# oxylusengine/Oxylus

Measured on NVIDIA H100. Metric: meshlet_instances_culled_per_s, higher is better.
Workload: dtype f32

## Files before the change

oxylus_b200/csrc/kernels_tri.cuh:

```cuda
#pragma once
#include <climits>

#include "oxc_exact.cuh"
#include "oxc_raster_core.cuh"
#include "oxc_tma.cuh"

namespace oxc {

#ifndef OXC_TRI_THREADS
#define OXC_TRI_THREADS 256
#endif
constexpr int TRI_THREADS = OXC_TRI_THREADS;
constexpr int TRI_WARPS = TRI_THREADS / 32;

struct TriParams {
  const OxcMeshletInstance* meshlet_instances;
  const InstCull* inst;
  const InstGeom* geom;
  const OxcMeshletInstanceVisibility* vis;
  const OxcDispatchIndirectCommand* tri_cmd;
  const uint32_t* visible_indices;
  const uint32_t* id_base;
  uint32_t late;
  uint32_t* reordered_indices;
// ... 72 lines not shown
  const uint32_t first = p.late ? p.vis->early_visible_meshlet_instances : 0u;
  const uint32_t count = p.tri_cmd->x;
  const uint32_t id_base = p.id_base ? __ldg(p.id_base) : 0u;
  const uint32_t n_tiles = (count + TRI_WARPS - 1) / TRI_WARPS;
  float4* clip_s = clip_all[warp];
  for (uint32_t tile = blockIdx.x; tile < n_tiles; tile += gridDim.x) {
    const uint32_t g = tile * TRI_WARPS + warp;
    bool pass[2] = {false, false};
    uint32_t rank[2] = {0, 0}, wtotal = 0, data_id = 0;
    if (g < count) {
      const MeshletWork w = load_meshlet(p, first + g, id_base, clip_s, lane);
      data_id = w.data_id;
#pragma unroll
      for (int k = 0; k < 2; k++) {
        const uint32_t t = lane + 32u * k;
        float4 c0, c1, c2;
        pass[k] = t < w.tri_count && triangle_passes(w, t, clip_s, c0, c1, c2);
        if (pass[k] && p.small_primitive_cull && tri_covers_no_sample(c0, c1, c2, p.f_width, p.f_height, p.width, p.height)) pass[k] = false;
        const uint32_t bal = __ballot_sync(0xffffffffu, pass[k]);
        rank[k] = wtotal + __popc(bal & ((1u << lane) - 1u));
        wtotal += __popc(bal);
      }
      __syncwarp();
    }
    if (lane == 0) warp_cnt[warp] = wtotal;
    __syncthreads();
    if (threadIdx.x == 0) {
      uint32_t s = 0;
#pragma unroll
      for (int k = 0; k < TRI_WARPS; k++) { const uint32_t c = warp_cnt[k]; warp_cnt[k] = s; s += c; }
      base_s = s ? atomicAdd(&p.draw_cmd->index_count, s * 3u) : 0u;
    }
    __syncthreads();
    const uint32_t wbase = base_s + warp_cnt[warp] * 3u;
#pragma unroll
    for (int k = 0; k < 2; k++)
      if (pass[k]) {
        const uint32_t t = lane + 32u * k, off = wbase + rank[k] * 3u, masked = data_id << OXC_VIS_PRIMITIVE_BITS;
        p.reordered_indices[off + 0] = masked | ((t * 3u + 0u) & OXC_VIS_PRIMITIVE_MASK);
        p.reordered_indices[off + 1] = masked | ((t * 3u + 1u) & OXC_VIS_PRIMITIVE_MASK);
        p.reordered_indices[off + 2] = masked | ((t * 3u + 2u) & OXC_VIS_PRIMITIVE_MASK);
      }
    __syncthreads();
  }
}

#ifndef OXC_RASTER_MIN_BLOCKS
#define OXC_RASTER_MIN_BLOCKS 3
#endif
#ifndef OXC_RASTER_BIG_PIXELS
#define OXC_RASTER_BIG_PIXELS 32
#endif
#ifndef OXC_RASTER_BATCH
#define OXC_RASTER_BATCH 8
#endif
constexpr int MICRO_STAGE_BYTES = 224;
constexpr int RASTER_BATCH = OXC_RASTER_BATCH;
static_assert(RASTER_BATCH >= 1 && RASTER_BATCH <= 32, "one header per lane: a grab holds at most 32 meshlets");
constexpr int RASTER_BIG_PIXELS = OXC_RASTER_BIG_PIXELS;

struct MeshletHeader {
  uint32_t gid, inst, vertex_offset, vertex_count, tri_offset, tri_count;
  const uint32_t* micro;
  const uint32_t* vidx;
  const uint2* pos;
};

OXC_DI MeshletHeader fetch_header(const TriParams& p, uint32_t slot, uint32_t id_base) {
  MeshletHeader h;
  h.gid = __ldg(&p.visible_indices[slot]);
  const uint2 mi = __ldg(reinterpret_cast<const uint2*>(p.meshlet_instances) + (h.gid - id_base));
  const InstGeom* g = p.geom + mi.x;
  const uint4 g0 = __ldg(reinterpret_cast<const uint4*>(g));
  const uint4 g1 = __ldg(reinterpret_cast<const uint4*>(g) + 1);
  const OxcMeshlet* meshlets = reinterpret_cast<const OxcMeshlet*>(((uint64_t)g0.y << 32) | g0.x);
  const uint4 m = __ldg(reinterpret_cast<const uint4*>(meshlets + mi.y));
  h.inst = mi.x;
  h.vertex_offset = m.x;
  h.tri_offset = m.y;
  h.vertex_count = min(m.z, (uint32_t)OXC_MESHLET_MAX_VERTICES);
  h.tri_count = min(m.w, (uint32_t)OXC_MESHLET_MAX_PRIMITIVES);
  h.micro = reinterpret_cast<const uint32_t*>(((uint64_t)g0.w << 32) | g0.z);
  h.vidx = reinterpret_cast<const uint32_t*>(((uint64_t)g1.y << 32) | g1.x) + m.x;
  h.pos = reinterpret_cast<const uint2*>(((uint64_t)g1.w << 32) | g1.z);
  return h;
}

OXC_DI MeshletHeader bcast_header(const MeshletHeader& h, int src) {
  MeshletHeader o;
  o.gid = __shfl_sync(0xffffffffu, h.gid, src); o.inst = __shfl_sync(0xffffffffu, h.inst, src);
  o.vertex_offset = 0;
  o.vertex_count = __shfl_sync(0xffffffffu, h.vertex_count, src);
  o.tri_offset = __shfl_sync(0xffffffffu, h.tri_offset, src); o.tri_count = __shfl_sync(0xffffffffu, h.tri_count, src);
  o.micro = reinterpret_cast<const uint32_t*>(__shfl_sync(0xffffffffu, reinterpret_cast<unsigned long long>(h.micro), src));
  o.vidx = reinterpret_cast<const uint32_t*>(__shfl_sync(0xffffffffu, reinterpret_cast<unsigned long long>(h.vidx), src));
  o.pos = reinterpret_cast<const uint2*>(__shfl_sync(0xffffffffu, reinterpret_cast<unsigned long long>(h.pos), src));
  return o;
}

constexpr int BIG_CHUNK_W = 64, BIG_CHUNK_H = 32;

OXC_DI void big_entry_store(uint4* dst, const TriSetup& s, int px0, int px1, int py0, int py1, uint32_t data) {
  dst[0] = make_uint4((uint32_t)s.ax, (uint32_t)s.ay, (uint32_t)s.bx, (uint32_t)s.by);
  dst[1] = make_uint4((uint32_t)s.cx, (uint32_t)s.cy, __float_as_uint(s.za), __float_as_uint(s.dzb));
  dst[2] = make_uint4(__float_as_uint(s.dzc), (uint32_t)px0, (uint32_t)px1, (uint32_t)py0);
  dst[3] = make_uint4((uint32_t)py1, (uint32_t)s.bias, data, 0u);
}

OXC_DI void big_entry_load(const uint4* src, TriSetup& s, uint32_t& data) {
  const uint4 a = src[0], b = src[1], c = src[2], d = src[3];
  s.ax = (int)a.x; s.ay = (int)a.y; s.bx = (int)a.z; s.by = (int)a.w;
  s.cx = (int)b.x; s.cy = (int)b.y; s.za = __uint_as_float(b.z); s.dzb = __uint_as_float(b.w);
  s.dzc = __uint_as_float(c.x); s.px0 = (int)c.y; s.px1 = (int)c.z; s.py0 = (int)c.w;
  s.py1 = (int)d.x; s.bias = (int)d.y; s.narrow = false;
  data = d.z;
}

OXC_DI bool big_push(const TriParams& p, const TriSetup& s, uint32_t data) {
  if (*reinterpret_cast<volatile uint32_t*>(&p.big_counters[0]) >= p.big_capacity) return false;
  const uint32_t cw = (uint32_t)(s.px1 - s.px0) / BIG_CHUNK_W + 1u, ch = (uint32_t)(s.py1 - s.py0) / BIG_CHUNK_H + 1u;
  const uint32_t n = cw * ch;
  const uint32_t base = atomicAdd(&p.big_counters[0], n);
  if (base >= p.big_capacity) return false;
  if (base + n > p.big_capacity) {
    for (uint32_t k = base; k < p.big_capacity; k++) big_entry_store(p.big_queue + (size_t)k * 4, s, 1, 0, 1, 0, data);
    return false;
  }
  uint32_t k = base;
  for (uint32_t cy = 0; cy < ch; cy++)
    for (uint32_t cx = 0; cx < cw; cx++, k++) {
      const int x0 = s.px0 + (int)(cx * BIG_CHUNK_W), y0 = s.py0 + (int)(cy * BIG_CHUNK_H);
      big_entry_store(p.big_queue + (size_t)k * 4, s, x0, min(s.px1, x0 + BIG_CHUNK_W - 1), y0, min(s.py1, y0 + BIG_CHUNK_H - 1), data);
    }
  return true;
}

constexpr uint32_t BIG_PUSH_ALONE = 4;
OXC_DI uint32_t big_chunk_count(const TriSetup& s) {
  return ((uint32_t)(s.px1 - s.px0) / BIG_CHUNK_W + 1u) * ((uint32_t)(s.py1 - s.py0) / BIG_CHUNK_H + 1u);
}

OXC_DI bool big_push_warp(const TriParams& p, const TriSetup& s, uint32_t data, uint32_t lane) {
  const uint32_t cw = (uint32_t)(s.px1 - s.px0) / BIG_CHUNK_W + 1u, ch = (uint32_t)(s.py1 - s.py0) / BIG_CHUNK_H + 1u;
  const uint32_t n = cw * ch;
  uint32_t base = 0xFFFFFFFFu;
  if (lane == 0 && *reinterpret_cast<volatile uint32_t*>(&p.big_counters[0]) < p.big_capacity) base = atomicAdd(&p.big_counters[0], n);
  base = __shfl_sync(0xffffffffu, base, 0);
  if (base >= p.big_capacity) return false;
  if (base + n > p.big_capacity) {
    for (uint32_t k = base + lane; k < p.big_capacity; k += 32) big_entry_store(p.big_queue + (size_t)k * 4, s, 1, 0, 1, 0, data);
    return false;
  }
  for (uint32_t k = lane; k < n; k += 32) {
    const uint32_t cy = k / cw, cx = k - cy * cw;
    const int x0 = s.px0 + (int)(cx * BIG_CHUNK_W), y0 = s.py0 + (int)(cy * BIG_CHUNK_H);
    big_entry_store(p.big_queue + (size_t)(base + k) * 4, s, x0, min(s.px1, x0 + BIG_CHUNK_W - 1), y0, min(s.py1, y0 + BIG_CHUNK_H - 1), data);
  }
  return true;
}

__global__ void __launch_bounds__(256) k_raster_big(const __grid_constant__ TriParams p) {
  const uint32_t lane = threadIdx.x & 31;
  const uint32_t total = min(p.big_counters[0], p.big_capacity);
  const int lx = lane & 7, ly = lane >> 3;
  for (uint32_t i = blockIdx.x * (blockDim.x >> 5) + (threadIdx.x >> 5); i < total; i += gridDim.x * (blockDim.x >> 5)) {
    TriSetup b;
    uint32_t data;
    big_entry_load(p.big_queue + (size_t)i * 4, b, data);
    for (int ty = b.py0; ty <= b.py1; ty += 4)
      for (int tx = b.px0; tx <= b.px1; tx += 8) {
        const int px = tx + lx, py = ty + ly;
        if (px <= b.px1 && py <= b.py1) raster_pixel(b, px, py, data, p.visbuf, p.width);
      }
  }
}

template <bool PREFETCH_GRAB>
__global__ void __launch_bounds__(TRI_THREADS, OXC_RASTER_MIN_BLOCKS) k_raster_visbuffer(const __grid_constant__ TriParams p) {
  __shared__ float4 clip_all[TRI_WARPS][OXC_MESHLET_MAX_VERTICES];
  __shared__ ScreenVert scr_all[TRI_WARPS][OXC_MESHLET_MAX_VERTICES];
  const uint32_t lane = threadIdx.x & 31, warp = threadIdx.x >> 5;
#ifndef OXC_RASTER_NO_SMEM_MICRO
#define OXC_RASTER_SMEM_MICRO 1
#endif
#ifdef OXC_RASTER_SMEM_MICRO
  __shared__ uint32_t micro_w[TRI_WARPS][52];
#endif
#ifdef OXC_RASTER_TMA_MICRO
  __shared__ __align__(16) uint8_t micro_all[TRI_WARPS][MICRO_STAGE_BYTES];
  __shared__ __align__(8) uint64_t micro_bar[TRI_WARPS];
  if (lane == 0) { mbar_init(&micro_bar[warp], 1); mbar_fence_init(); }
  __syncwarp();
  uint32_t micro_phase = 0;
#endif
  const uint32_t first = p.late ? p.vis->early_visible_meshlet_instances : 0u;
  const uint32_t count = p.tri_cmd->x;
  const uint32_t id_base = p.id_base ? __ldg(p.id_base) : 0u;
  float4* clip_s = clip_all[warp];
  ScreenVert* scr_s = scr_all[warp];
  uint32_t kept = 0;
#ifdef OXC_RASTER_STATS
  unsigned long long t_entry, t_chase = 0, t_proc = 0, n_done = 0, n_grabs = 0;
  asm volatile("mov.u64 %0, %%globaltimer;" : "=l"(t_entry));
#endif
  const uint32_t n_warps2 = gridDim.x * TRI_WARPS * 2u;
  uint32_t g_next = 0, batch_next = 1;
  if (PREFETCH_GRAB && lane == 0) {
    batch_next = min((uint32_t)RASTER_BATCH, max(1u, count / n_warps2));
    g_next = atomicAdd(p.work_counter, batch_next);
  }
  for (;;) {
    uint32_t g0 = 0, batch = 1;
    if (PREFETCH_GRAB) {
      g0 = __shfl_sync(0xffffffffu, g_next, 0);
      batch = __shfl_sync(0xffffffffu, batch_next, 0);
      if (g0 >= count) break;
      if (lane == 0) {
        const uint32_t seen = g0 + batch;
        const uint32_t rem = count > seen ? count - seen : 0u;
        batch_next = min((uint32_t)RASTER_BATCH, max(1u, rem / n_warps2));
        g_next = atomicAdd(p.work_counter, batch_next);
      }
    } else {
      if (lane == 0) {
        const uint32_t seen = *reinterpret_cast<volatile uint32_t*>(p.work_counter);
        const uint32_t rem = count > seen ? count - seen : 0u;
        batch = min((uint32_t)RASTER_BATCH, max(1u, rem / n_warps2));
        g0 = atomicAdd(p.work_counter, batch);
      }
      g0 = __shfl_sync(0xffffffffu, g0, 0);
      batch = __shfl_sync(0xffffffffu, batch, 0);
      if (g0 >= count) break;
    }
    const uint32_t nb = min(batch, count - g0);
    const uint32_t my_survivor = g0 + lane;
#ifdef OXC_RASTER_STATS
    unsigned long long t_a, t_b, t_c;
    asm volatile("mov.u64 %0, %%globaltimer;" : "=l"(t_a));
#endif
    MeshletHeader mine;
    mine.gid = 0; mine.inst = 0; mine.vertex_offset = 0; mine.vertex_count = 0; mine.tri_offset = 0; mine.tri_count = 0;
    mine.micro = nullptr; mine.vidx = nullptr; mine.pos = nullptr;
    if (lane < nb) mine = fetch_header(p, first + my_survivor, id_base);
    MeshletHeader cur = bcast_header(mine, 0);
    uint32_t vi0 = lane < cur.vertex_count ? __ldg(&cur.vidx[lane]) : 0u;
    uint32_t vi1 = lane + 32u < cur.vertex_count ? __ldg(&cur.vidx[lane + 32u]) : 0u;
#ifdef OXC_RASTER_STATS
    if (vi0 + vi1 == 0xFFFFFFFFu) kept++;
    asm volatile("mov.u64 %0, %%globaltimer;" : "=l"(t_b));
#endif
    for (uint32_t j = 0; j < nb; j++) {
      const MeshletHeader w = cur;
#ifdef OXC_RASTER_TMA_MICRO
      const uint64_t micro_addr = reinterpret_cast<uint64_t>(w.micro) + w.tri_offset;
      const uint32_t micro_skew = (uint32_t)(micro_addr & 15u);
      if (lane == 0) {
        const uint32_t bytes = (micro_skew + w.tri_count * 3u + 15u) & ~15u;
        mbar_expect_tx(&micro_bar[warp], bytes);
        tma_load_1d(micro_all[warp], reinterpret_cast<const void*>(micro_addr - micro_skew), bytes, &micro_bar[warp]);
      }
#endif
#ifdef OXC_RASTER_SMEM_MICRO
      {
        const uint32_t n_words = ((w.tri_offset & 3u) + w.tri_count * 3u + 3u) >> 2;
        const uint32_t* src = w.micro + (w.tri_offset >> 2);
        const uint32_t m0 = lane < n_words ? __ldg(src + lane) : 0u;
        const uint32_t m1 = lane + 32u < n_words ? __ldg(src + lane + 32u) : 0u;
        micro_w[warp][lane] = m0;
        if (lane < 20) micro_w[warp][lane + 32] = m1;
      }
#endif
      const uint2 q0 = lane < w.vertex_count ? __ldg(&w.pos[vi0]) : make_uint2(0, 0);
      const uint2 q1 = lane + 32u < w.vertex_count ? __ldg(&w.pos[vi1]) : make_uint2(0, 0);
      if (j + 1 < nb) {
        cur = bcast_header(mine, (int)(j + 1));
        vi0 = lane < cur.vertex_count ? __ldg(&cur.vidx[lane]) : 0u;
        vi1 = lane + 32u < cur.vertex_count ? __ldg(&cur.vidx[lane + 32u]) : 0u;
      }
      const InstCull* ic = p.inst + w.inst;
      const float4 r0 = __ldg(&ic->mvp_row[0]), r1 = __ldg(&ic->mvp_row[1]), r2 = __ldg(&ic->mvp_row[2]), r3 = __ldg(&ic->mvp_row[3]);
      {
        const float x = dequantize_half_hw(q0.x & 0xFFFFu), y = dequantize_half_hw(q0.x >> 16), z = dequantize_half_hw(q0.y & 0xFFFFu);
        const float4 c = make_float4(row_dot_p1(r0, x, y, z), row_dot_p1(r1, x, y, z), row_dot_p1(r2, x, y, z), row_dot_p1(r3, x, y, z));
        clip_s[lane] = c;
        scr_s[lane] = to_screen(c, p.f_width, p.f_height);
      }
      if (w.vertex_count > 32u) {
        const float x = dequantize_half_hw(q1.x & 0xFFFFu), y = dequantize_half_hw(q1.x >> 16), z = dequantize_half_hw(q1.y & 0xFFFFu);
        const float4 c = make_float4(row_dot_p1(r0, x, y, z), row_dot_p1(r1, x, y, z), row_dot_p1(r2, x, y, z), row_dot_p1(r3, x, y, z));
        clip_s[lane + 32] = c;
        scr_s[lane + 32] = to_screen(c, p.f_width, p.f_height);
      }
      __syncwarp();
#ifdef OXC_RASTER_TMA_MICRO
      mbar_wait(&micro_bar[warp], micro_phase);
      micro_phase ^= 1u;
      const uint8_t* micro_s = micro_all[warp] + micro_skew;
#endif
      const uint32_t rounds = (w.tri_count + 31u) >> 5;
      for (uint32_t k = 0; k < rounds; k++) {
        const uint32_t t = lane + 32u * k;
        bool pass = false;
        TriSetup s;
        bool draw = false;
        if (t < w.tri_count) {
#ifdef OXC_RASTER_TMA_MICRO
          const uint32_t i0 = micro_s[t * 3u + 0u], i1 = micro_s[t * 3u + 1u], i2 = micro_s[t * 3u + 2u];
#elif defined(OXC_RASTER_SMEM_MICRO)
          const uint8_t* mb = reinterpret_cast<const uint8_t*>(micro_w[warp]) + (w.tri_offset & 3u) + t * 3u;
          const uint32_t i0 = mb[0], i1 = mb[1], i2 = mb[2];
#else
          const uint32_t base = w.tri_offset + t * 3u;
          const uint32_t i0 = micro_index(w.micro, base + 0u), i1 = micro_index(w.micro, base + 1u), i2 = micro_index(w.micro, base + 2u);
#endif
          if (max(i0, max(i1, i2)) < w.vertex_count) {
            const float4 c0 = clip_s[i0], c1 = clip_s[i1], c2 = clip_s[i2];
            pass = c0.z >= 0.0f && c1.z >= 0.0f && c2.z >= 0.0f && !triangle_backface(c0, c1, c2);
            if (pass) {
              const int why = tri_setup(scr_s[i0], scr_s[i1], scr_s[i2], p.width, p.height, s);
              draw = why == TRI_DRAW;
              if (why == TRI_NO_SAMPLE && p.small_primitive_cull) pass = false;
              if (why == TRI_INVALID_VERTEX && p.clip_queue) {
                const uint32_t slot = atomicAdd(p.clip_counter, 1u);
                if (slot < p.clip_capacity) p.clip_queue[slot] = (w.gid << p.prim_bits) | t;
                else atomicOr(p.status, (uint32_t)OXC_STATUS_CLIP_OVERFLOW);
              }
            }
          }
        }
        kept += pass ? 1u : 0u;
        const uint32_t data = (w.gid << p.prim_bits) | t;
        const int bw = draw ? s.px1 - s.px0 + 1 : 0, bh = draw ? s.py1 - s.py0 + 1 : 0;
#if defined(OXC_RASTER_STATS) && OXC_RASTER_STATS == 1
        {
          const int area = (draw && bw * bh <= RASTER_BIG_PIXELS) ? bw * bh : 0;
          const int mx = __reduce_max_sync(0xffffffffu, area), sm = __reduce_add_sync(0xffffffffu, area);
          const int nd = __popc(__ballot_sync(0xffffffffu, area > 0));
          const int nbig = __popc(__ballot_sync(0xffffffffu, draw && bw * bh > RASTER_BIG_PIXELS));
          if (lane == 0) {
            unsigned long long* st = reinterpret_cast<unsigned long long*>(p.big_queue) + (size_t)p.big_capacity * 8 + (p.late ? 64 : 0);
            atomicAdd(&st[min(mx, 33)], 1ull);
            atomicAdd(&st[40], (unsigned long long)sm);
            atomicAdd(&st[41], (unsigned long long)mx);
            atomicAdd(&st[42], (unsigned long long)nd);
            atomicAdd(&st[43], 1ull);
            atomicAdd(&st[44], (unsigned long long)nbig);
          }
        }
#endif
        bool big = draw && (bw * bh > RASTER_BIG_PIXELS);
        if (draw && !big) raster_small(s, data, p.visbuf, p.width);
        const bool few = big && big_chunk_count(s) <= BIG_PUSH_ALONE;
        if (few && p.big_queue && big_push(p, s, data)) big = false;
        uint32_t big_mask = __ballot_sync(0xffffffffu, big);
        while (big_mask) {
          const int src = __ffs(big_mask) - 1;
          big_mask &= big_mask - 1;
          TriSetup b;
          b.ax = __shfl_sync(0xffffffffu, s.ax, src); b.ay = __shfl_sync(0xffffffffu, s.ay, src);
          b.bx = __shfl_sync(0xffffffffu, s.bx, src); b.by = __shfl_sync(0xffffffffu, s.by, src);
          b.cx = __shfl_sync(0xffffffffu, s.cx, src); b.cy = __shfl_sync(0xffffffffu, s.cy, src);
          b.za = __shfl_sync(0xffffffffu, s.za, src); b.dzb = __shfl_sync(0xffffffffu, s.dzb, src);
          b.dzc = __shfl_sync(0xffffffffu, s.dzc, src);
          b.px0 = __shfl_sync(0xffffffffu, s.px0, src); b.px1 = __shfl_sync(0xffffffffu, s.px1, src);
          b.py0 = __shfl_sync(0xffffffffu, s.py0, src); b.py1 = __shfl_sync(0xffffffffu, s.py1, src);
          b.bias = __shfl_sync(0xffffffffu, s.bias, src);
          const uint32_t bdata = __shfl_sync(0xffffffffu, data, src);
          if (p.big_queue && big_push_warp(p, b, bdata, lane)) continue;
          const int lx = lane & 7, ly = lane >> 3;
          for (int ty = b.py0; ty <= b.py1; ty += 4)
            for (int tx = b.px0; tx <= b.px1; tx += 8) {
              const int px = tx + lx, py = ty + ly;
              if (px <= b.px1 && py <= b.py1) raster_pixel(b, px, py, bdata, p.visbuf, p.width);
            }
        }
      }
      __syncwarp();
    }
#ifdef OXC_RASTER_STATS
    asm volatile("mov.u64 %0, %%globaltimer;" : "=l"(t_c));
    t_chase += t_b - t_a; t_proc += t_c - t_b; n_done += nb; n_grabs++;
#endif
  }
#ifdef OXC_RASTER_STATS
  if (lane == 0) {
    unsigned long long t_exit;
    asm volatile("mov.u64 %0, %%globaltimer;" : "=l"(t_exit));
    unsigned long long* rec = reinterpret_cast<unsigned long long*>(p.big_queue) + (size_t)p.big_capacity * 8 + 128 +
                              ((size_t)(p.late ? gridDim.x * TRI_WARPS : 0) + blockIdx.x * TRI_WARPS + warp) * 6;
    rec[0] = t_entry; rec[1] = t_exit; rec[2] = t_chase; rec[3] = t_proc; rec[4] = n_done; rec[5] = n_grabs;
    if (blockIdx.x == 0 && warp == 0)
      reinterpret_cast<unsigned long long*>(p.big_queue)[(size_t)p.big_capacity * 8 + (p.late ? 64 : 0) + 45] = gridDim.x;
  }
#endif
#pragma unroll
  for (int o = 16; o > 0; o >>= 1) kept += __shfl_xor_sync(0xffffffffu, kept, o);
  if (lane == 0 && kept) atomicAdd(p.tri_counter, (unsigned long long)kept);
}

OXC_DI void clip_and_draw(const TriParams& p, float4 c0, float4 c1, float4 c2, uint32_t data, float fW, float fH) {
  float4 poly[2][12];
  int cur;
  const int n = clip_polygon(c0, c1, c2, poly, cur);
  for (int i = 1; i + 1 < n; i++) {
    TriSetup s;
    if (tri_setup(to_screen(poly[cur][0], fW, fH), to_screen(poly[cur][i], fW, fH), to_screen(poly[cur][i + 1], fW, fH), p.width, p.height, s) != TRI_DRAW)
      continue;
    const int bw = s.px1 - s.px0 + 1, bh = s.py1 - s.py0 + 1;
    if (bw * bh > RASTER_BIG_PIXELS && p.big_queue && big_push(p, s, data)) continue;
    s.narrow = false;
    raster_small(s, data, p.visbuf, p.width);
  }
}

__global__ void __launch_bounds__(128) k_raster_clip_queue(const __grid_constant__ TriParams p) {
  const uint32_t n = min(*p.clip_counter, p.clip_capacity);
  const uint32_t id_base = p.id_base ? __ldg(p.id_base) : 0u;
  for (uint32_t e = blockIdx.x * blockDim.x + threadIdx.x; e < n; e += gridDim.x * blockDim.x) {
    const uint32_t data = p.clip_queue[e];
    const uint32_t gid = data >> p.prim_bits, t = data & ((1u << p.prim_bits) - 1u);
    const uint2 mi = __ldg(reinterpret_cast<const uint2*>(p.meshlet_instances) + (gid - id_base));
    const InstGeom* g = p.geom + mi.x;
    const InstCull* ic = p.inst + mi.x;
    const uint4 m = __ldg(reinterpret_cast<const uint4*>(g->meshlets + mi.y));
    const float4 r0 = __ldg(&ic->mvp_row[0]), r1 = __ldg(&ic->mvp_row[1]), r2 = __ldg(&ic->mvp_row[2]), r3 = __ldg(&ic->mvp_row[3]);
    float4 c[3];
#pragma unroll
    for (int k = 0; k < 3; k++) {
      const uint32_t li = micro_index(g->local_triangle_indices, m.y + t * 3u + k);
      const uint32_t vi = __ldg(&g->indirect_vertex_indices[m.x + li]);
      const uint2 q = __ldg(&g->vertex_positions[vi]);
      const float x = dequantize_half_hw(q.x & 0xFFFFu), y = dequantize_half_hw(q.x >> 16), z = dequantize_half_hw(q.y & 0xFFFFu);
      c[k] = make_float4(row_dot_p1(r0, x, y, z), row_dot_p1(r1, x, y, z), row_dot_p1(r2, x, y, z), row_dot_p1(r3, x, y, z));
    }
    clip_and_draw(p, c[0], c[1], c[2], data, p.f_width, p.f_height);
// ... 55 lines not shown
```

oxylus_b200/csrc/oxc_raster_core.cuh:

```cuda
#pragma once
#include <climits>

#include "oxc_exact.cuh"

namespace oxc {

struct __align__(16) ScreenVert {
  int fx, fy;
  float z;
  int pad;
};

OXC_DI ScreenVert to_screen(float4 c, float fW, float fH) {
  ScreenVert v;
  v.fx = INT_MIN; v.fy = 0; v.z = 0.f; v.pad = 0;
  if (!(c.w > 0.0f)) return v;
  const float rw = fd(1.0f, c.w);
  const float nx = fm(c.x, rw), ny = fm(c.y, rw);
  const float sx = fm(fa(fm(nx, 0.5f), 0.5f), fW), sy = fm(fa(fm(ny, 0.5f), 0.5f), fH);
  const float qx = floorf(fa(fm(sx, 256.0f), 0.5f)), qy = floorf(fa(fm(sy, 256.0f), 0.5f));
  if (!(fabsf(qx) <= 4194304.0f && fabsf(qy) <= 4194304.0f)) return v;
  v.fx = (int)qx; v.fy = (int)qy; v.z = fm(c.z, rw);
  return v;
}

OXC_DI bool tri_covers_no_sample(float4 c0, float4 c1, float4 c2, float fW, float fH, uint32_t W, uint32_t H) {
  const ScreenVert v0 = to_screen(c0, fW, fH), v1 = to_screen(c1, fW, fH), v2 = to_screen(c2, fW, fH);
  if (v0.fx == INT_MIN || v1.fx == INT_MIN || v2.fx == INT_MIN) return false;
  const int minx = min(v0.fx, min(v1.fx, v2.fx)), maxx = max(v0.fx, max(v1.fx, v2.fx));
  const int miny = min(v0.fy, min(v1.fy, v2.fy)), maxy = max(v0.fy, max(v1.fy, v2.fy));
  const int px0 = max(0, (minx - 128 + 255) >> 8), px1 = min((int)W - 1, (maxx - 128) >> 8);
  const int py0 = max(0, (miny - 128 + 255) >> 8), py1 = min((int)H - 1, (maxy - 128) >> 8);
  return px1 < px0 || py1 < py0;
}

struct TriSetup {
  int ax, ay, bx, by, cx, cy;
  float za, dzb, dzc;
  int px0, px1, py0, py1;
  int bias;
  bool narrow;
};

OXC_DI long long orient2d(int ax, int ay, int bx, int by, int cx, int cy) {
  return (long long)(bx - ax) * (long long)(cy - ay) - (long long)(by - ay) * (long long)(cx - ax);
}
OXC_DI int edge_bias_bit(int ax, int ay, int bx, int by) {
  const int dx = bx - ax, dy = by - ay;
  return ((dy > 0) || (dy == 0 && dx < 0)) ? 0 : 1;
}

enum : int { TRI_DRAW = 0, TRI_INVALID_VERTEX = 1, TRI_NO_SAMPLE = 2, TRI_BACK_OR_DEGENERATE = 3 };
OXC_DI int tri_setup(const ScreenVert v0, const ScreenVert v1, const ScreenVert v2, uint32_t W, uint32_t H, TriSetup& s) {
  if (v0.fx == INT_MIN || v1.fx == INT_MIN || v2.fx == INT_MIN) return TRI_INVALID_VERTEX;
  const int minx = min(v0.fx, min(v1.fx, v2.fx)), maxx = max(v0.fx, max(v1.fx, v2.fx));
  const int miny = min(v0.fy, min(v1.fy, v2.fy)), maxy = max(v0.fy, max(v1.fy, v2.fy));
  s.px0 = max(0, (minx - 128 + 255) >> 8);
  s.px1 = min((int)W - 1, (maxx - 128) >> 8);
  s.py0 = max(0, (miny - 128 + 255) >> 8);
  s.py1 = min((int)H - 1, (maxy - 128) >> 8);
  if (s.px1 < s.px0 || s.py1 < s.py0) return TRI_NO_SAMPLE;
  s.narrow = (maxx - minx) < 16384 && (maxy - miny) < 16384;
  long long area2;
  if (s.narrow) area2 = (long long)((v1.fx - v0.fx) * (v2.fy - v0.fy) - (v1.fy - v0.fy) * (v2.fx - v0.fx));
  else area2 = orient2d(v0.fx, v0.fy, v1.fx, v1.fy, v2.fx, v2.fy);
  if (area2 >= 0) return TRI_BACK_OR_DEGENERATE;
  s.ax = v0.fx; s.ay = v0.fy; s.bx = v2.fx; s.by = v2.fy; s.cx = v1.fx; s.cy = v1.fy;
  const float fa_ = (float)(-area2);
  s.za = v0.z;
  s.dzb = fd(fs(v2.z, v0.z), fa_);
  s.dzc = fd(fs(v1.z, v0.z), fa_);
  s.bias = edge_bias_bit(s.bx, s.by, s.cx, s.cy) | (edge_bias_bit(s.cx, s.cy, s.ax, s.ay) << 1) |
           (edge_bias_bit(s.ax, s.ay, s.bx, s.by) << 2);
  return TRI_DRAW;
}

OXC_DI void shade_pixel(const TriSetup& s, long long e0, long long e1, long long e2, int px, int py, uint32_t data,
                        unsigned long long* vis, uint32_t W) {
  if ((e0 - (s.bias & 1)) < 0 || (e1 - ((s.bias >> 1) & 1)) < 0 || (e2 - ((s.bias >> 2) & 1)) < 0) return;
  const float zz = fa(fa(s.za, fm((float)e1, s.dzb)), fm((float)e2, s.dzc));
  if (!(zz >= 0.0f && zz <= 1.0f)) return;
  uint32_t zb = __float_as_uint(zz);
  zb = zb == 0x80000000u ? 0u : zb;
  const unsigned long long v = ((unsigned long long)zb << 32) | data;
  unsigned long long* ptr = vis + (size_t)py * W + px;
  atomicMax(ptr, v);
}

OXC_DI void raster_pixel(const TriSetup& s, int px, int py, uint32_t data, unsigned long long* vis, uint32_t W) {
  const int sx = px * 256 + 128, sy = py * 256 + 128;
  shade_pixel(s, orient2d(s.bx, s.by, s.cx, s.cy, sx, sy), orient2d(s.cx, s.cy, s.ax, s.ay, sx, sy),
              orient2d(s.ax, s.ay, s.bx, s.by, sx, sy), px, py, data, vis, W);
}

OXC_DI int orient2d_32(int ax, int ay, int bx, int by, int cx, int cy) { return (bx - ax) * (cy - ay) - (by - ay) * (cx - ax); }

OXC_DI void shade_pixel_32(const TriSetup& s, int e0, int e1, int e2, int px, int py, uint32_t data, unsigned long long* vis,
                           uint32_t W) {
  if ((e0 - (s.bias & 1)) < 0 || (e1 - ((s.bias >> 1) & 1)) < 0 || (e2 - ((s.bias >> 2) & 1)) < 0) return;
  const float zz = fa(fa(s.za, fm((float)e1, s.dzb)), fm((float)e2, s.dzc));
  if (!(zz >= 0.0f && zz <= 1.0f)) return;
  uint32_t zb = __float_as_uint(zz);
  zb = zb == 0x80000000u ? 0u : zb;
  const unsigned long long v = ((unsigned long long)zb << 32) | data;
  unsigned long long* ptr = vis + (size_t)py * W + px;
  atomicMax(ptr, v);
}

OXC_DI void raster_small(const TriSetup& s, uint32_t data, unsigned long long* vis, uint32_t W) {
  const int sx0 = s.px0 * 256 + 128, sy0 = s.py0 * 256 + 128;
  if (s.narrow) {
    int r0 = orient2d_32(s.bx, s.by, s.cx, s.cy, sx0, sy0), r1 = orient2d_32(s.cx, s.cy, s.ax, s.ay, sx0, sy0),
        r2 = orient2d_32(s.ax, s.ay, s.bx, s.by, sx0, sy0);
    const int dx0 = -(s.cy - s.by) * 256, dy0 = (s.cx - s.bx) * 256, dx1 = -(s.ay - s.cy) * 256, dy1 = (s.ax - s.cx) * 256,
              dx2 = -(s.by - s.ay) * 256, dy2 = (s.bx - s.ax) * 256;
    for (int py = s.py0; py <= s.py1; py++) {
      int e0 = r0, e1 = r1, e2 = r2;
      for (int px = s.px0; px <= s.px1; px++) {
        shade_pixel_32(s, e0, e1, e2, px, py, data, vis, W);
        e0 += dx0; e1 += dx1; e2 += dx2;
      }
      r0 += dy0; r1 += dy1; r2 += dy2;
    }
    return;
  }
  long long r0 = orient2d(s.bx, s.by, s.cx, s.cy, sx0, sy0);
  long long r1 = orient2d(s.cx, s.cy, s.ax, s.ay, sx0, sy0);
  long long r2 = orient2d(s.ax, s.ay, s.bx, s.by, sx0, sy0);
  const long long dx0 = -(long long)(s.cy - s.by) * 256, dy0 = (long long)(s.cx - s.bx) * 256;
  const long long dx1 = -(long long)(s.ay - s.cy) * 256, dy1 = (long long)(s.ax - s.cx) * 256;
  const long long dx2 = -(long long)(s.by - s.ay) * 256, dy2 = (long long)(s.bx - s.ax) * 256;
  for (int py = s.py0; py <= s.py1; py++) {
    long long e0 = r0, e1 = r1, e2 = r2;
    for (int px = s.px0; px <= s.px1; px++) {
      shade_pixel(s, e0, e1, e2, px, py, data, vis, W);
      e0 += dx0; e1 += dx1; e2 += dx2;
    }
    r0 += dy0; r1 += dy1; r2 += dy2;
  }
}

OXC_DI float clip_plane_distance(const float4 v, int plane) {
  switch (plane) {
    case 0: return fs(v.w, v.z);
    case 1: return fa(v.w, v.x);
    case 2: return fs(v.w, v.x);
    case 3: return fa(v.w, v.y);
    default: return fs(v.w, v.y);
  }
}

OXC_DI int clip_polygon(float4 c0, float4 c1, float4 c2, float4 (*poly)[12], int& cur) {
  int n = 3;
  cur = 0;
  poly[0][0] = c0; poly[0][1] = c1; poly[0][2] = c2;
  for (int plane = 0; plane < 5 && n >= 3; plane++) {
    const float4* in = poly[cur];
    float4* out = poly[cur ^ 1];
    int m = 0;
    for (int i = 0; i < n; i++) {
      const float4 A = in[i], B = in[(i + 1) % n];
      const float dA = clip_plane_distance(A, plane), dB = clip_plane_distance(B, plane);
      const bool inA = dA >= 0.0f, inB = dB >= 0.0f;
      if (inA) out[m++] = A;
      if (inA != inB) {
        const float4 I = inA ? A : B, O = inA ? B : A;
        const float dI = inA ? dA : dB, dO = inA ? dB : dA;
        const float tt = fd(dI, fs(dI, dO));
        out[m++] = make_float4(fa(I.x, fm(tt, fs(O.x, I.x))), fa(I.y, fm(tt, fs(O.y, I.y))), fa(I.z, fm(tt, fs(O.z, I.z))),
                               fa(I.w, fm(tt, fs(O.w, I.w))));
      }
    }
    n = m;
    cur ^= 1;
  }
  return n;
}

// ... 2 lines not shown
```

Baseline: 1.808 billion.

## Compact drawable triangles into per-warp shared queue before rasterizing

Drawable triangles are no longer rasterized in the same lane that classified them. Their screen vertices go into a per-warp shared-memory queue, and rasterization starts only once 32 are queued, so all lanes stay busy instead of idling on rounds where few triangles survive. Meshlet headers now live in shared memory instead of being broadcast with shuffles, triangle setup is split into decide and finish steps, and the grab batch size doubles. The cost is more shared memory per block, which could lower occupancy, setup work repeated when triangles leave the queue, and pixel writes that may occur in a different order.

```diff
diff --git a/oxylus_b200/csrc/kernels_tri.cuh b/oxylus_b200/csrc/kernels_tri.cuh
--- a/oxylus_b200/csrc/kernels_tri.cuh
+++ b/oxylus_b200/csrc/kernels_tri.cuh
@@ -148,7 +148,7 @@
 #define OXC_RASTER_BIG_PIXELS 32
 #endif
 #ifndef OXC_RASTER_BATCH
-#define OXC_RASTER_BATCH 8
+#define OXC_RASTER_BATCH 16
 #endif
 constexpr int MICRO_STAGE_BYTES = 224;
 constexpr int RASTER_BATCH = OXC_RASTER_BATCH;
@@ -182,18 +182,6 @@
   return h;
 }
 
-OXC_DI MeshletHeader bcast_header(const MeshletHeader& h, int src) {
-  MeshletHeader o;
-  o.gid = __shfl_sync(0xffffffffu, h.gid, src); o.inst = __shfl_sync(0xffffffffu, h.inst, src);
-  o.vertex_offset = 0;
-  o.vertex_count = __shfl_sync(0xffffffffu, h.vertex_count, src);
-  o.tri_offset = __shfl_sync(0xffffffffu, h.tri_offset, src); o.tri_count = __shfl_sync(0xffffffffu, h.tri_count, src);
-  o.micro = reinterpret_cast<const uint32_t*>(__shfl_sync(0xffffffffu, reinterpret_cast<unsigned long long>(h.micro), src));
-  o.vidx = reinterpret_cast<const uint32_t*>(__shfl_sync(0xffffffffu, reinterpret_cast<unsigned long long>(h.vidx), src));
-  o.pos = reinterpret_cast<const uint2*>(__shfl_sync(0xffffffffu, reinterpret_cast<unsigned long long>(h.pos), src));
-  return o;
-}
-
 constexpr int BIG_CHUNK_W = 64, BIG_CHUNK_H = 32;
 
 OXC_DI void big_entry_store(uint4* dst, const TriSetup& s, int px0, int px1, int py0, int py1, uint32_t data) {
@@ -271,10 +259,87 @@
   }
 }
 
+#ifdef OXC_RASTER_STATS
+OXC_DI unsigned long long* raster_stats_slots(const TriParams& p) {
+  return reinterpret_cast<unsigned long long*>(p.big_queue) + (size_t)p.big_capacity * 8 + (p.late ? 64 : 0);
+}
+#endif
+
+constexpr int RASTER_QUEUE = 64;
+struct RasterQueue {
+  ScreenVert v[3][RASTER_QUEUE];
+};
+
+OXC_DI void queue_store(RasterQueue& q, uint32_t i, ScreenVert v0, const ScreenVert v1, const ScreenVert v2, uint32_t data) {
+  v0.pad = (int)data;
+  q.v[0][i] = v0; q.v[1][i] = v1; q.v[2][i] = v2;
+}
+
+OXC_DI void queue_setup(const RasterQueue& q, uint32_t i, uint32_t W, uint32_t H, TriSetup& s, uint32_t& data) {
+  const ScreenVert v0 = q.v[0][i], v1 = q.v[1][i], v2 = q.v[2][i];
+  long long area2;
+  tri_decide(v0, v1, v2, W, H, s, area2);
+  tri_finish(v0, v1, v2, area2, s);
+  data = (uint32_t)v0.pad;
+}
+
+OXC_DI void raster_queued(const TriParams& p, const RasterQueue& q, uint32_t base, uint32_t cnt, uint32_t lane) {
+  const bool draw = lane < cnt;
+  TriSetup s;
+  uint32_t data = 0;
+  int bw = 0, bh = 0;
+  if (draw) {
+    queue_setup(q, base + lane, p.width, p.height, s, data);
+    bw = s.px1 - s.px0 + 1; bh = s.py1 - s.py0 + 1;
+  }
+#ifdef OXC_RASTER_STATS
+  {
+    unsigned long long* st = raster_stats_slots(p);
+#if OXC_RASTER_STATS == 1
+    const int area = (draw && bw * bh <= RASTER_BIG_PIXELS) ? bw * bh : 0;
+    const int mx = __reduce_max_sync(0xffffffffu, area), sm = __reduce_add_sync(0xffffffffu, area);
+    const int nbig = __popc(__ballot_sync(0xffffffffu, draw && bw * bh > RASTER_BIG_PIXELS));
+    if (lane == 0) {
+      atomicAdd(&st[min(mx, 33)], 1ull);
+      atomicAdd(&st[40], (unsigned long long)sm);
+      atomicAdd(&st[41], (unsigned long long)mx);
+      atomicAdd(&st[44], (unsigned long long)nbig);
+    }
+#endif
+    if (lane == 0) {
+      atomicAdd(&st[46], 1ull);
+      atomicAdd(&st[47], (unsigned long long)cnt);
+    }
+  }
+#endif
+  bool big = draw && (bw * bh > RASTER_BIG_PIXELS);
+  if (draw && !big) raster_small(s, data, p.visbuf, p.width);
+  const bool few = big && big_chunk_count(s) <= BIG_PUSH_ALONE;
+  if (few && p.big_queue && big_push(p, s, data)) big = false;
+  uint32_t big_mask = __ballot_sync(0xffffffffu, big);
+  while (big_mask) {
+    const int src = __ffs(big_mask) - 1;
+    big_mask &= big_mask - 1;
+    TriSetup b;
+    uint32_t bdata;
+    queue_setup(q, base + src, p.width, p.height, b, bdata);
+    if (p.big_queue && big_push_warp(p, b, bdata, lane)) continue;
+    const int lx = lane & 7, ly = lane >> 3;
+    for (int ty = b.py0; ty <= b.py1; ty += 4)
+      for (int tx = b.px0; tx <= b.px1; tx += 8) {
+        const int px = tx + lx, py = ty + ly;
+        if (px <= b.px1 && py <= b.py1) raster_pixel(b, px, py, bdata, p.visbuf, p.width);
+      }
+  }
+  __syncwarp();
+}
+
 template <bool PREFETCH_GRAB>
 __global__ void __launch_bounds__(TRI_THREADS, OXC_RASTER_MIN_BLOCKS) k_raster_visbuffer(const __grid_constant__ TriParams p) {
   __shared__ float4 clip_all[TRI_WARPS][OXC_MESHLET_MAX_VERTICES];
   __shared__ ScreenVert scr_all[TRI_WARPS][OXC_MESHLET_MAX_VERTICES];
+  __shared__ MeshletHeader hdr_all[TRI_WARPS][RASTER_BATCH];
+  __shared__ RasterQueue queue_all[TRI_WARPS];
   const uint32_t lane = threadIdx.x & 31, warp = threadIdx.x >> 5;
 #ifndef OXC_RASTER_NO_SMEM_MICRO
 #define OXC_RASTER_SMEM_MICRO 1
@@ -294,6 +359,9 @@
   const uint32_t id_base = p.id_base ? __ldg(p.id_base) : 0u;
   float4* clip_s = clip_all[warp];
   ScreenVert* scr_s = scr_all[warp];
+  MeshletHeader* hdr_s = hdr_all[warp];
+  RasterQueue& q = queue_all[warp];
+  uint32_t queued = 0;
   uint32_t kept = 0;
 #ifdef OXC_RASTER_STATS
   unsigned long long t_entry, t_chase = 0, t_proc = 0, n_done = 0, n_grabs = 0;
@@ -334,19 +402,16 @@
     unsigned long long t_a, t_b, t_c;
     asm volatile("mov.u64 %0, %%globaltimer;" : "=l"(t_a));
 #endif
-    MeshletHeader mine;
-    mine.gid = 0; mine.inst = 0; mine.vertex_offset = 0; mine.vertex_count = 0; mine.tri_offset = 0; mine.tri_count = 0;
-    mine.micro = nullptr; mine.vidx = nullptr; mine.pos = nullptr;
-    if (lane < nb) mine = fetch_header(p, first + my_survivor, id_base);
-    MeshletHeader cur = bcast_header(mine, 0);
-    uint32_t vi0 = lane < cur.vertex_count ? __ldg(&cur.vidx[lane]) : 0u;
-    uint32_t vi1 = lane + 32u < cur.vertex_count ? __ldg(&cur.vidx[lane + 32u]) : 0u;
+    if (lane < nb) hdr_s[lane] = fetch_header(p, first + my_survivor, id_base);
+    __syncwarp();
+    uint32_t vi0 = lane < hdr_s[0].vertex_count ? __ldg(&hdr_s[0].vidx[lane]) : 0u;
+    uint32_t vi1 = lane + 32u < hdr_s[0].vertex_count ? __ldg(&hdr_s[0].vidx[lane + 32u]) : 0u;
 #ifdef OXC_RASTER_STATS
     if (vi0 + vi1 == 0xFFFFFFFFu) kept++;
     asm volatile("mov.u64 %0, %%globaltimer;" : "=l"(t_b));
 #endif
     for (uint32_t j = 0; j < nb; j++) {
-      const MeshletHeader w = cur;
+      const MeshletHeader& w = hdr_s[j];
 #ifdef OXC_RASTER_TMA_MICRO
       const uint64_t micro_addr = reinterpret_cast<uint64_t>(w.micro) + w.tri_offset;
       const uint32_t micro_skew = (uint32_t)(micro_addr & 15u);
@@ -369,9 +434,9 @@
       const uint2 q0 = lane < w.vertex_count ? __ldg(&w.pos[vi0]) : make_uint2(0, 0);
       const uint2 q1 = lane + 32u < w.vertex_count ? __ldg(&w.pos[vi1]) : make_uint2(0, 0);
       if (j + 1 < nb) {
-        cur = bcast_header(mine, (int)(j + 1));
-        vi0 = lane < cur.vertex_count ? __ldg(&cur.vidx[lane]) : 0u;
-        vi1 = lane + 32u < cur.vertex_count ? __ldg(&cur.vidx[lane + 32u]) : 0u;
+        const MeshletHeader& next = hdr_s[j + 1];
+        vi0 = lane < next.vertex_count ? __ldg(&next.vidx[lane]) : 0u;
+        vi1 = lane + 32u < next.vertex_count ? __ldg(&next.vidx[lane + 32u]) : 0u;
       }
       const InstCull* ic = p.inst + w.inst;
       const float4 r0 = __ldg(&ic->mvp_row[0]), r1 = __ldg(&ic->mvp_row[1]), r2 = __ldg(&ic->mvp_row[2]), r3 = __ldg(&ic->mvp_row[3]);
@@ -397,7 +462,7 @@
       for (uint32_t k = 0; k < rounds; k++) {
         const uint32_t t = lane + 32u * k;
         bool pass = false;
-        TriSetup s;
+        uint32_t corners = 0;
         bool draw = false;
         if (t < w.tri_count) {
 #ifdef OXC_RASTER_TMA_MICRO
@@ -413,7 +478,10 @@
             const float4 c0 = clip_s[i0], c1 = clip_s[i1], c2 = clip_s[i2];
             pass = c0.z >= 0.0f && c1.z >= 0.0f && c2.z >= 0.0f && !triangle_backface(c0, c1, c2);
             if (pass) {
-              const int why = tri_setup(scr_s[i0], scr_s[i1], scr_s[i2], p.width, p.height, s);
+              corners = i0 | i1 << 8 | i2 << 16;
+              TriSetup s;
+              long long area2;
+              const int why = tri_decide(scr_s[i0], scr_s[i1], scr_s[i2], p.width, p.height, s, area2);
               draw = why == TRI_DRAW;
               if (why == TRI_NO_SAMPLE && p.small_primitive_cull) pass = false;
               if (why == TRI_INVALID_VERTEX && p.clip_queue) {
@@ -425,50 +493,22 @@
           }
         }
         kept += pass ? 1u : 0u;
-        const uint32_t data = (w.gid << p.prim_bits) | t;
-        const int bw = draw ? s.px1 - s.px0 + 1 : 0, bh = draw ? s.py1 - s.py0 + 1 : 0;
+        const uint32_t drawn = __ballot_sync(0xffffffffu, draw);
 #if defined(OXC_RASTER_STATS) && OXC_RASTER_STATS == 1
-        {
-          const int area = (draw && bw * bh <= RASTER_BIG_PIXELS) ? bw * bh : 0;
-          const int mx = __reduce_max_sync(0xffffffffu, area), sm = __reduce_add_sync(0xffffffffu, area);
-          const int nd = __popc(__ballot_sync(0xffffffffu, area > 0));
-          const int nbig = __popc(__ballot_sync(0xffffffffu, draw && bw * bh > RASTER_BIG_PIXELS));
-          if (lane == 0) {
-            unsigned long long* st = reinterpret_cast<unsigned long long*>(p.big_queue) + (size_t)p.big_capacity * 8 + (p.late ? 64 : 0);
-            atomicAdd(&st[min(mx, 33)], 1ull);
-            atomicAdd(&st[40], (unsigned long long)sm);
-            atomicAdd(&st[41], (unsigned long long)mx);
-            atomicAdd(&st[42], (unsigned long long)nd);
-            atomicAdd(&st[43], 1ull);
-            atomicAdd(&st[44], (unsigned long long)nbig);
-          }
+        if (lane == 0) {
+          unsigned long long* st = raster_stats_slots(p);
+          atomicAdd(&st[42], (unsigned long long)__popc(drawn));
+          atomicAdd(&st[43], 1ull);
         }
 #endif
-        bool big = draw && (bw * bh > RASTER_BIG_PIXELS);
-        if (draw && !big) raster_small(s, data, p.visbuf, p.width);
-        const bool few = big && big_chunk_count(s) <= BIG_PUSH_ALONE;
-        if (few && p.big_queue && big_push(p, s, data)) big = false;
-        uint32_t big_mask = __ballot_sync(0xffffffffu, big);
-        while (big_mask) {
-          const int src = __ffs(big_mask) - 1;
-          big_mask &= big_mask - 1;
-          TriSetup b;
-          b.ax = __shfl_sync(0xffffffffu, s.ax, src); b.ay = __shfl_sync(0xffffffffu, s.ay, src);
-          b.bx = __shfl_sync(0xffffffffu, s.bx, src); b.by = __shfl_sync(0xffffffffu, s.by, src);
-          b.cx = __shfl_sync(0xffffffffu, s.cx, src); b.cy = __shfl_sync(0xffffffffu, s.cy, src);
-          b.za = __shfl_sync(0xffffffffu, s.za, src); b.dzb = __shfl_sync(0xffffffffu, s.dzb, src);
-          b.dzc = __shfl_sync(0xffffffffu, s.dzc, src);
-          b.px0 = __shfl_sync(0xffffffffu, s.px0, src); b.px1 = __shfl_sync(0xffffffffu, s.px1, src);
-          b.py0 = __shfl_sync(0xffffffffu, s.py0, src); b.py1 = __shfl_sync(0xffffffffu, s.py1, src);
-          b.bias = __shfl_sync(0xffffffffu, s.bias, src);
-          const uint32_t bdata = __shfl_sync(0xffffffffu, data, src);
-          if (p.big_queue && big_push_warp(p, b, bdata, lane)) continue;
-          const int lx = lane & 7, ly = lane >> 3;
-          for (int ty = b.py0; ty <= b.py1; ty += 4)
-            for (int tx = b.px0; tx <= b.px1; tx += 8) {
-              const int px = tx + lx, py = ty + ly;
-              if (px <= b.px1 && py <= b.py1) raster_pixel(b, px, py, bdata, p.visbuf, p.width);
-            }
+        if (draw)
+          queue_store(q, queued + __popc(drawn & ((1u << lane) - 1u)), scr_s[corners & 0xFFu], scr_s[(corners >> 8) & 0xFFu],
+                      scr_s[corners >> 16], (w.gid << p.prim_bits) | t);
+        queued += __popc(drawn);
+        if (queued >= 32u) {
+          __syncwarp();
+          queued -= 32u;
+          raster_queued(p, q, queued, 32u, lane);
         }
       }
       __syncwarp();
@@ -477,6 +517,10 @@
     asm volatile("mov.u64 %0, %%globaltimer;" : "=l"(t_c));
     t_chase += t_b - t_a; t_proc += t_c - t_b; n_done += nb; n_grabs++;
 #endif
+  }
+  if (queued) {
+    __syncwarp();
+    raster_queued(p, q, 0u, queued, lane);
   }
 #ifdef OXC_RASTER_STATS
   if (lane == 0) {
diff --git a/oxylus_b200/csrc/oxc_raster_core.cuh b/oxylus_b200/csrc/oxc_raster_core.cuh
--- a/oxylus_b200/csrc/oxc_raster_core.cuh
+++ b/oxylus_b200/csrc/oxc_raster_core.cuh
@@ -51,6 +51,34 @@
 }
 
 enum : int { TRI_DRAW = 0, TRI_INVALID_VERTEX = 1, TRI_NO_SAMPLE = 2, TRI_BACK_OR_DEGENERATE = 3 };
+
+OXC_DI int tri_decide(const ScreenVert v0, const ScreenVert v1, const ScreenVert v2, uint32_t W, uint32_t H, TriSetup& s,
+                      long long& area2) {
+  if (v0.fx == INT_MIN || v1.fx == INT_MIN || v2.fx == INT_MIN) return TRI_INVALID_VERTEX;
+  const int minx = min(v0.fx, min(v1.fx, v2.fx)), maxx = max(v0.fx, max(v1.fx, v2.fx));
+  const int miny = min(v0.fy, min(v1.fy, v2.fy)), maxy = max(v0.fy, max(v1.fy, v2.fy));
+  s.px0 = max(0, (minx - 128 + 255) >> 8);
+  s.px1 = min((int)W - 1, (maxx - 128) >> 8);
+  s.py0 = max(0, (miny - 128 + 255) >> 8);
+  s.py1 = min((int)H - 1, (maxy - 128) >> 8);
+  if (s.px1 < s.px0 || s.py1 < s.py0) return TRI_NO_SAMPLE;
+  s.narrow = (maxx - minx) < 16384 && (maxy - miny) < 16384;
+  if (s.narrow) area2 = (long long)((v1.fx - v0.fx) * (v2.fy - v0.fy) - (v1.fy - v0.fy) * (v2.fx - v0.fx));
+  else area2 = orient2d(v0.fx, v0.fy, v1.fx, v1.fy, v2.fx, v2.fy);
+  if (area2 >= 0) return TRI_BACK_OR_DEGENERATE;
+  return TRI_DRAW;
+}
+
+OXC_DI void tri_finish(const ScreenVert v0, const ScreenVert v1, const ScreenVert v2, long long area2, TriSetup& s) {
+  s.ax = v0.fx; s.ay = v0.fy; s.bx = v2.fx; s.by = v2.fy; s.cx = v1.fx; s.cy = v1.fy;
+  const float fa_ = (float)(-area2);
+  s.za = v0.z;
+  s.dzb = fd(fs(v2.z, v0.z), fa_);
+  s.dzc = fd(fs(v1.z, v0.z), fa_);
+  s.bias = edge_bias_bit(s.bx, s.by, s.cx, s.cy) | (edge_bias_bit(s.cx, s.cy, s.ax, s.ay) << 1) |
+           (edge_bias_bit(s.ax, s.ay, s.bx, s.by) << 2);
+}
+
 OXC_DI int tri_setup(const ScreenVert v0, const ScreenVert v1, const ScreenVert v2, uint32_t W, uint32_t H, TriSetup& s) {
   if (v0.fx == INT_MIN || v1.fx == INT_MIN || v2.fx == INT_MIN) return TRI_INVALID_VERTEX;
   const int minx = min(v0.fx, min(v1.fx, v2.fx)), maxx = max(v0.fx, max(v1.fx, v2.fx));
```

After: 1.903 billion (median of 6 runs). 1.05x the previous value.

## Stage meshlet headers in shared memory and route wide small triangles to big path

Applied to the files above, without the earlier changes.

Per-lane meshlet headers are now written to a per-warp shared-memory array and read back by index, replacing shuffle-based broadcasts that kept a full header live in registers. Small-triangle rasterization is restricted to the 32-bit narrow path, and non-narrow triangles are sent to the big/binned path so the 64-bit edge loop leaves the hot inline code. This aims to cut register pressure and shuffle overhead in the raster kernel. In exchange it adds shared-memory traffic and more big-queue work for wide triangles.

```diff
diff --git a/oxylus_b200/csrc/kernels_tri.cuh b/oxylus_b200/csrc/kernels_tri.cuh
--- a/oxylus_b200/csrc/kernels_tri.cuh
+++ b/oxylus_b200/csrc/kernels_tri.cuh
@@ -155,12 +155,13 @@
 static_assert(RASTER_BATCH >= 1 && RASTER_BATCH <= 32, "one header per lane: a grab holds at most 32 meshlets");
 constexpr int RASTER_BIG_PIXELS = OXC_RASTER_BIG_PIXELS;
 
-struct MeshletHeader {
-  uint32_t gid, inst, vertex_offset, vertex_count, tri_offset, tri_count;
+struct __align__(16) MeshletHeader {
+  uint32_t gid, inst, vertex_count, tri_offset, tri_count;
   const uint32_t* micro;
   const uint32_t* vidx;
   const uint2* pos;
 };
+static_assert(sizeof(MeshletHeader) == 48, "three 128-bit words");
 
 OXC_DI MeshletHeader fetch_header(const TriParams& p, uint32_t slot, uint32_t id_base) {
   MeshletHeader h;
@@ -172,7 +173,6 @@
   const OxcMeshlet* meshlets = reinterpret_cast<const OxcMeshlet*>(((uint64_t)g0.y << 32) | g0.x);
   const uint4 m = __ldg(reinterpret_cast<const uint4*>(meshlets + mi.y));
   h.inst = mi.x;
-  h.vertex_offset = m.x;
   h.tri_offset = m.y;
   h.vertex_count = min(m.z, (uint32_t)OXC_MESHLET_MAX_VERTICES);
   h.tri_count = min(m.w, (uint32_t)OXC_MESHLET_MAX_PRIMITIVES);
@@ -180,18 +180,6 @@
   h.vidx = reinterpret_cast<const uint32_t*>(((uint64_t)g1.y << 32) | g1.x) + m.x;
   h.pos = reinterpret_cast<const uint2*>(((uint64_t)g1.w << 32) | g1.z);
   return h;
-}
-
-OXC_DI MeshletHeader bcast_header(const MeshletHeader& h, int src) {
-  MeshletHeader o;
-  o.gid = __shfl_sync(0xffffffffu, h.gid, src); o.inst = __shfl_sync(0xffffffffu, h.inst, src);
-  o.vertex_offset = 0;
-  o.vertex_count = __shfl_sync(0xffffffffu, h.vertex_count, src);
-  o.tri_offset = __shfl_sync(0xffffffffu, h.tri_offset, src); o.tri_count = __shfl_sync(0xffffffffu, h.tri_count, src);
-  o.micro = reinterpret_cast<const uint32_t*>(__shfl_sync(0xffffffffu, reinterpret_cast<unsigned long long>(h.micro), src));
-  o.vidx = reinterpret_cast<const uint32_t*>(__shfl_sync(0xffffffffu, reinterpret_cast<unsigned long long>(h.vidx), src));
-  o.pos = reinterpret_cast<const uint2*>(__shfl_sync(0xffffffffu, reinterpret_cast<unsigned long long>(h.pos), src));
-  return o;
 }
 
 constexpr int BIG_CHUNK_W = 64, BIG_CHUNK_H = 32;
@@ -275,6 +263,7 @@
 __global__ void __launch_bounds__(TRI_THREADS, OXC_RASTER_MIN_BLOCKS) k_raster_visbuffer(const __grid_constant__ TriParams p) {
   __shared__ float4 clip_all[TRI_WARPS][OXC_MESHLET_MAX_VERTICES];
   __shared__ ScreenVert scr_all[TRI_WARPS][OXC_MESHLET_MAX_VERTICES];
+  __shared__ MeshletHeader hdr_all[TRI_WARPS][RASTER_BATCH];
   const uint32_t lane = threadIdx.x & 31, warp = threadIdx.x >> 5;
 #ifndef OXC_RASTER_NO_SMEM_MICRO
 #define OXC_RASTER_SMEM_MICRO 1
@@ -294,6 +283,7 @@
   const uint32_t id_base = p.id_base ? __ldg(p.id_base) : 0u;
   float4* clip_s = clip_all[warp];
   ScreenVert* scr_s = scr_all[warp];
+  MeshletHeader* hdr_s = hdr_all[warp];
   uint32_t kept = 0;
 #ifdef OXC_RASTER_STATS
   unsigned long long t_entry, t_chase = 0, t_proc = 0, n_done = 0, n_grabs = 0;
@@ -329,24 +319,20 @@
       if (g0 >= count) break;
     }
     const uint32_t nb = min(batch, count - g0);
-    const uint32_t my_survivor = g0 + lane;
 #ifdef OXC_RASTER_STATS
     unsigned long long t_a, t_b, t_c;
     asm volatile("mov.u64 %0, %%globaltimer;" : "=l"(t_a));
 #endif
-    MeshletHeader mine;
-    mine.gid = 0; mine.inst = 0; mine.vertex_offset = 0; mine.vertex_count = 0; mine.tri_offset = 0; mine.tri_count = 0;
-    mine.micro = nullptr; mine.vidx = nullptr; mine.pos = nullptr;
-    if (lane < nb) mine = fetch_header(p, first + my_survivor, id_base);
-    MeshletHeader cur = bcast_header(mine, 0);
-    uint32_t vi0 = lane < cur.vertex_count ? __ldg(&cur.vidx[lane]) : 0u;
-    uint32_t vi1 = lane + 32u < cur.vertex_count ? __ldg(&cur.vidx[lane + 32u]) : 0u;
+    if (lane < nb) hdr_s[lane] = fetch_header(p, first + g0 + lane, id_base);
+    __syncwarp();
+    uint32_t vi0 = lane < hdr_s[0].vertex_count ? __ldg(&hdr_s[0].vidx[lane]) : 0u;
+    uint32_t vi1 = lane + 32u < hdr_s[0].vertex_count ? __ldg(&hdr_s[0].vidx[lane + 32u]) : 0u;
 #ifdef OXC_RASTER_STATS
     if (vi0 + vi1 == 0xFFFFFFFFu) kept++;
     asm volatile("mov.u64 %0, %%globaltimer;" : "=l"(t_b));
 #endif
     for (uint32_t j = 0; j < nb; j++) {
-      const MeshletHeader w = cur;
+      const MeshletHeader w = hdr_s[j];
 #ifdef OXC_RASTER_TMA_MICRO
       const uint64_t micro_addr = reinterpret_cast<uint64_t>(w.micro) + w.tri_offset;
       const uint32_t micro_skew = (uint32_t)(micro_addr & 15u);
@@ -369,9 +355,9 @@
       const uint2 q0 = lane < w.vertex_count ? __ldg(&w.pos[vi0]) : make_uint2(0, 0);
       const uint2 q1 = lane + 32u < w.vertex_count ? __ldg(&w.pos[vi1]) : make_uint2(0, 0);
       if (j + 1 < nb) {
-        cur = bcast_header(mine, (int)(j + 1));
-        vi0 = lane < cur.vertex_count ? __ldg(&cur.vidx[lane]) : 0u;
-        vi1 = lane + 32u < cur.vertex_count ? __ldg(&cur.vidx[lane + 32u]) : 0u;
+        const MeshletHeader& n = hdr_s[j + 1];
+        vi0 = lane < n.vertex_count ? __ldg(&n.vidx[lane]) : 0u;
+        vi1 = lane + 32u < n.vertex_count ? __ldg(&n.vidx[lane + 32u]) : 0u;
       }
       const InstCull* ic = p.inst + w.inst;
       const float4 r0 = __ldg(&ic->mvp_row[0]), r1 = __ldg(&ic->mvp_row[1]), r2 = __ldg(&ic->mvp_row[2]), r3 = __ldg(&ic->mvp_row[3]);
@@ -427,12 +413,13 @@
         kept += pass ? 1u : 0u;
         const uint32_t data = (w.gid << p.prim_bits) | t;
         const int bw = draw ? s.px1 - s.px0 + 1 : 0, bh = draw ? s.py1 - s.py0 + 1 : 0;
+        bool big = draw && (!s.narrow || bw * bh > RASTER_BIG_PIXELS);
 #if defined(OXC_RASTER_STATS) && OXC_RASTER_STATS == 1
         {
-          const int area = (draw && bw * bh <= RASTER_BIG_PIXELS) ? bw * bh : 0;
+          const int area = (draw && !big) ? bw * bh : 0;
           const int mx = __reduce_max_sync(0xffffffffu, area), sm = __reduce_add_sync(0xffffffffu, area);
           const int nd = __popc(__ballot_sync(0xffffffffu, area > 0));
-          const int nbig = __popc(__ballot_sync(0xffffffffu, draw && bw * bh > RASTER_BIG_PIXELS));
+          const int nbig = __popc(__ballot_sync(0xffffffffu, big));
           if (lane == 0) {
             unsigned long long* st = reinterpret_cast<unsigned long long*>(p.big_queue) + (size_t)p.big_capacity * 8 + (p.late ? 64 : 0);
             atomicAdd(&st[min(mx, 33)], 1ull);
@@ -444,8 +431,7 @@
           }
         }
 #endif
-        bool big = draw && (bw * bh > RASTER_BIG_PIXELS);
-        if (draw && !big) raster_small(s, data, p.visbuf, p.width);
+        if (draw && !big) raster_small_narrow(s, data, p.visbuf, p.width);
         const bool few = big && big_chunk_count(s) <= BIG_PUSH_ALONE;
         if (few && p.big_queue && big_push(p, s, data)) big = false;
         uint32_t big_mask = __ballot_sync(0xffffffffu, big);
diff --git a/oxylus_b200/csrc/oxc_raster_core.cuh b/oxylus_b200/csrc/oxc_raster_core.cuh
--- a/oxylus_b200/csrc/oxc_raster_core.cuh
+++ b/oxylus_b200/csrc/oxc_raster_core.cuh
@@ -107,23 +107,28 @@
   atomicMax(ptr, v);
 }
 
+OXC_DI void raster_small_narrow(const TriSetup& s, uint32_t data, unsigned long long* vis, uint32_t W) {
+  const int sx0 = s.px0 * 256 + 128, sy0 = s.py0 * 256 + 128;
+  int r0 = orient2d_32(s.bx, s.by, s.cx, s.cy, sx0, sy0), r1 = orient2d_32(s.cx, s.cy, s.ax, s.ay, sx0, sy0),
+      r2 = orient2d_32(s.ax, s.ay, s.bx, s.by, sx0, sy0);
+  const int dx0 = -(s.cy - s.by) * 256, dy0 = (s.cx - s.bx) * 256, dx1 = -(s.ay - s.cy) * 256, dy1 = (s.ax - s.cx) * 256,
+            dx2 = -(s.by - s.ay) * 256, dy2 = (s.bx - s.ax) * 256;
+  for (int py = s.py0; py <= s.py1; py++) {
+    int e0 = r0, e1 = r1, e2 = r2;
+    for (int px = s.px0; px <= s.px1; px++) {
+      shade_pixel_32(s, e0, e1, e2, px, py, data, vis, W);
+      e0 += dx0; e1 += dx1; e2 += dx2;
+    }
+    r0 += dy0; r1 += dy1; r2 += dy2;
+  }
+}
+
 OXC_DI void raster_small(const TriSetup& s, uint32_t data, unsigned long long* vis, uint32_t W) {
-  const int sx0 = s.px0 * 256 + 128, sy0 = s.py0 * 256 + 128;
   if (s.narrow) {
-    int r0 = orient2d_32(s.bx, s.by, s.cx, s.cy, sx0, sy0), r1 = orient2d_32(s.cx, s.cy, s.ax, s.ay, sx0, sy0),
-        r2 = orient2d_32(s.ax, s.ay, s.bx, s.by, sx0, sy0);
-    const int dx0 = -(s.cy - s.by) * 256, dy0 = (s.cx - s.bx) * 256, dx1 = -(s.ay - s.cy) * 256, dy1 = (s.ax - s.cx) * 256,
-              dx2 = -(s.by - s.ay) * 256, dy2 = (s.bx - s.ax) * 256;
-    for (int py = s.py0; py <= s.py1; py++) {
-      int e0 = r0, e1 = r1, e2 = r2;
-      for (int px = s.px0; px <= s.px1; px++) {
-        shade_pixel_32(s, e0, e1, e2, px, py, data, vis, W);
-        e0 += dx0; e1 += dx1; e2 += dx2;
-      }
-      r0 += dy0; r1 += dy1; r2 += dy2;
-    }
+    raster_small_narrow(s, data, vis, W);
     return;
   }
+  const int sx0 = s.px0 * 256 + 128, sy0 = s.py0 * 256 + 128;
   long long r0 = orient2d(s.bx, s.by, s.cx, s.cy, sx0, sy0);
   long long r1 = orient2d(s.cx, s.cy, s.ax, s.ay, sx0, sy0);
   long long r2 = orient2d(s.ax, s.ay, s.bx, s.by, sx0, sy0);
```

Result: faster. 1.807 billion before, 1.841 billion after (median of 6 runs) (+1.9%).
